# pyannote/pyannote-audio

Measured on NVIDIA H100. Metric: audio-hours/sec (RTF) community-1 diarization, 16kHz mono, 1/2/4/8 H100, higher is better.
Workload: dtype f16 tensor-core trunk (f32 accumulate) + split-f16x3 tensor-core segmentation (f32-level accuracy) + f64 clustering

## Files before the change

pyannote_audio_b200/csrc/emb_conv.cu:

```cuda
#include "common.cuh"
#include "emb.cuh"
#include "tc_common.cuh"

namespace b200 {

constexpr int kWgThreads = 288;
constexpr int kTileM = 128;
constexpr int kRowHalo = 8;
constexpr int kMaxSlots = 16;

template <int N, bool WIDE = false>
__device__ __forceinline__ void conv_epilogue(const float* acc, const ConvParams& p, size_t row, int w0) {
  const int lane = threadIdx.x & 31;
  const int c0 = 2 * (lane & 3) + (WIDE ? (int)blockIdx.y * N : 0);
#pragma unroll
  for (int i = 0; i < 2; ++i) {
    const int w = w0 + ((threadIdx.x >> 5) & 3) * 16 + (lane >> 2) + 8 * i;
    if (w >= p.W_out) continue;
    const size_t pix = (row * p.W_out + w) * (size_t)(WIDE ? p.C_out : N);
    __half2 res[N / 8];
    if (N <= 64 && p.residual) {
#pragma unroll
      for (int j = 0; j < N / 8; ++j) res[j] = *reinterpret_cast<const __half2*>(p.residual + pix + 8 * j + c0);
    }
#pragma unroll
    for (int j = 0; j < N / 8; ++j) {
      const int c = 8 * j + c0;
      const float2 bb = __ldg(reinterpret_cast<const float2*>(p.bias + c));
      float a = acc[4 * j + 2 * i] + bb.x, d = acc[4 * j + 2 * i + 1] + bb.y;
      if (p.residual) {
        const float2 r = __half22float2(N <= 64 ? res[j] : *reinterpret_cast<const __half2*>(p.residual + pix + c));
        a += r.x;
        d += r.y;
      }
      if (p.relu) { a = fmaxf(a, 0.f); d = fmaxf(d, 0.f); }
      *reinterpret_cast<__half2*>(p.out + pix + c) = __floats2half2_rn(a, d);
    }
  }
}

template <int N, int CK, bool WIDE = false>
__global__ void __launch_bounds__(kWgThreads, N == 256 ? 1 : 2)
conv_tc_kernel(const __grid_constant__ CUtensorMap tmA, const __grid_constant__ CUtensorMap tmB, ConvParams p) {
  extern __shared__ uint8_t smem_raw[];
  const uint32_t raw = smem_u32(smem_raw);
  const uint32_t base = (raw + 1023u) & ~1023u;
  const uint32_t bar_full = base, bar_empty = base + 64;
  const uint32_t stage0 = base + 1024;
  const uint32_t stage_bytes = p.a_bytes + p.b_bytes;
  const int warp = threadIdx.x >> 5;
  const int wt = blockIdx.x % p.tiles_w;
  const int bh = blockIdx.x / p.tiles_w;
  const int cchunks = p.C_in / CK;

  if (threadIdx.x == 0) {
    for (uint32_t s = 0; s < p.nstages; ++s) { mbar_init(bar_full + 8 * s, 1); mbar_init(bar_empty + 8 * s, 2); }
    asm volatile("fence.mbarrier_init.release.cluster;" ::: "memory");
  }
  __syncthreads();

  if (warp == 8) {
    if ((threadIdx.x & 31) == 0) {
      prefetch_tensormap(&tmA);
      prefetch_tensormap(&tmB);
      const int h = bh % p.H_out, b = bh / p.H_out;
      const int w_base = wt * kTileM * p.stride - p.pad, h_base = h * p.stride - p.pad;
      uint32_t stage = 0, phase = 0;
      for (int kh = 0; kh < p.taps_h; ++kh)
        for (int kw = 0; kw < p.taps_w; ++kw)
          for (int cc = 0; cc < cchunks; ++cc) {
            mbar_wait(bar_empty + 8 * stage, phase ^ 1);
            mbar_expect_tx(bar_full + 8 * stage, p.a_tx + p.b_bytes);
            const uint32_t sa = stage0 + stage * stage_bytes;
            tma_load_4d(&tmA, bar_full + 8 * stage, sa, cc * CK, w_base + kw, h_base + kh, b);
            tma_load_3d(&tmB, bar_full + 8 * stage, sa + p.a_bytes, cc * CK, WIDE ? (int)blockIdx.y * N : 0,
                        kh * p.taps_w + kw);
            if (++stage == p.nstages) { stage = 0; phase ^= 1; }
          }
    }
    return;
  }

  const int wg = warp >> 2;
  constexpr uint32_t row_bytes = CK * 2;
  float acc[N / 2];
#pragma unroll
  for (int i = 0; i < N / 2; ++i) acc[i] = 0.f;
  const int kblocks = p.taps_h * p.taps_w * cchunks;
  uint32_t stage = 0, phase = 0, prev = 0;
  for (int kb = 0; kb < kblocks; ++kb) {
    mbar_wait(bar_full + 8 * stage, phase);
    const uint32_t st = stage0 + stage * stage_bytes;
    const uint32_t sa = st + (uint32_t)wg * 64u * row_bytes, sb = st + p.a_bytes;
    wg_fence();
    const uint64_t ad = wg_desc(sa, row_bytes), bd = wg_desc(sb, row_bytes);
#pragma unroll
    for (int k = 0; k < CK / 16; ++k) Wgmma<N>::mma(acc, ad + 2 * k, bd + 2 * k);
    wg_commit();
    wg_wait<1>();
    if (kb > 0 && (threadIdx.x & 127) == 0) mbar_arrive(bar_empty + 8 * prev);
    prev = stage;
    if (++stage == p.nstages) { stage = 0; phase ^= 1; }
  }
  wg_wait<0>();
  conv_epilogue<N, WIDE>(acc, p, (size_t)bh, wt * kTileM + wg * 64);
}

template <int N>
__device__ __forceinline__ void row_taps_c32(float (&acc)[2][N / 2], uint32_t sa, uint32_t wts) {
  constexpr uint32_t row_bytes = 64;
  const int warp = threadIdx.x >> 5, lane = threadIdx.x & 31;
#pragma unroll
  for (int kw = 0; kw < 3; ++kw) {
    uint32_t af[2][2][4];
#pragma unroll
    for (int m = 0; m < 2; ++m)
#pragma unroll
      for (int k = 0; k < 2; ++k) {
        const uint32_t row = (uint32_t)(m * 64 + (warp & 3) * 16 + (lane & 15) + kw);
        const uint32_t chunk = (uint32_t)(2 * k + (lane >> 4)) ^ ((row >> 1) & 3u);
        ldsm_x4(af[m][k], sa + row * row_bytes + chunk * 16u);
      }
    wg_fence();
    const uint64_t bd = wg_desc(wts + kw * N * row_bytes, row_bytes);
#pragma unroll
    for (int k = 0; k < 2; ++k)
#pragma unroll
      for (int m = 0; m < 2; ++m) WgmmaRS<N>::mma(acc[m], af[m][k], bd + 2 * k);
    wg_commit();
    wg_wait<0>();
  }
}

template <int N, int CK>
__global__ void __launch_bounds__(kWgThreads, N == 32 ? 2 : 1)
conv_row_kernel(const __grid_constant__ CUtensorMap tmA, const __grid_constant__ CUtensorMap tmB, ConvParams p) {
  constexpr uint32_t row_bytes = CK * 2;
  constexpr uint32_t b_tap_bytes = N * row_bytes;
  extern __shared__ uint8_t smem_raw[];
  const uint32_t base = (smem_u32(smem_raw) + 1023u) & ~1023u;
  const uint32_t bar_w = base, bar_full = base + 8, bar_empty = base + 8 + 8 * kMaxSlots;
  const uint32_t wts = base + 1024;
  const uint32_t slot0 = wts + 9 * b_tap_bytes;
  const uint32_t nslots = p.nstages;
  const int warp = threadIdx.x >> 5;

  if (threadIdx.x == 0) {
    mbar_init(bar_w, 1);
    for (uint32_t s = 0; s < nslots; ++s) { mbar_init(bar_full + 8 * s, 1); mbar_init(bar_empty + 8 * s, 3); }
    asm volatile("fence.mbarrier_init.release.cluster;" ::: "memory");
  }
  __syncthreads();

  if (warp == 8) {
    if ((threadIdx.x & 31) == 0) {
      prefetch_tensormap(&tmA);
      prefetch_tensormap(&tmB);
      mbar_expect_tx(bar_w, 9 * b_tap_bytes);
      for (int kh = 0; kh < 3; ++kh) tma_load_3d(&tmB, bar_w, wts + 3 * kh * b_tap_bytes, 0, 0, 3 * kh);
      uint32_t s = 0;
      for (int u = blockIdx.x; u < p.num_tiles; u += gridDim.x) {
        const int wt = u % p.tiles_w, t = u / p.tiles_w;
        const int h0 = (t % p.bands) * p.band, b = t / p.bands;
        const int n = min(p.band, p.H_out - h0);
        for (int r = 0; r < n + 2; ++r, ++s) {
          const uint32_t slot = s % nslots;
          mbar_wait(bar_empty + 8 * slot, ((s / nslots) & 1) ^ 1);
          mbar_expect_tx(bar_full + 8 * slot, p.a_tx);
          tma_load_4d(&tmA, bar_full + 8 * slot, slot0 + slot * p.a_bytes, 0, wt * kTileM - 1, h0 - 1 + r, b);
        }
      }
    }
    return;
  }

  const int wg = __shfl_sync(0xffffffffu, warp >> 2, 0);
  mbar_wait(bar_w, 0);
  uint32_t s = 0;
  int item = 0;
  for (int u = blockIdx.x; u < p.num_tiles; u += gridDim.x) {
    const int wt = u % p.tiles_w, t = u / p.tiles_w;
    const int h0 = (t % p.bands) * p.band, b = t / p.bands;
    const int n = min(p.band, p.H_out - h0);
    for (int j = 0; j < n; ++j, ++item) {
      if ((item & 1) != wg) continue;
      float acc[2][N / 2];
#pragma unroll
      for (int m = 0; m < 2; ++m)
#pragma unroll
        for (int i = 0; i < N / 2; ++i) {
          acc[m][i] = 0.f;
          asm volatile("" : "+f"(acc[m][i]));
        }
#pragma unroll
      for (int kh = 0; kh < 3; ++kh) {
        const uint32_t q = s + j + kh, slot = q % nslots;
        mbar_wait(bar_full + 8 * slot, (q / nslots) & 1);
        const uint32_t sa = slot0 + slot * p.a_bytes;
        if constexpr (CK == 32) {
          row_taps_c32<N>(acc, sa, wts + 3 * kh * b_tap_bytes);
        } else {
          wg_fence();
#pragma unroll
          for (int kw = 0; kw < 3; ++kw) {
            const uint64_t bd = wg_desc(wts + (3 * kh + kw) * b_tap_bytes, row_bytes);
#pragma unroll
            for (int m = 0; m < 2; ++m) {
              const uint64_t ad = wg_desc(sa + (uint32_t)(m * 64 + kw) * row_bytes, row_bytes);
#pragma unroll
              for (int k = 0; k < CK / 16; ++k) Wgmma<N>::mma(acc[m], ad + 2 * k, bd + 2 * k);
            }
          }
          wg_commit();
        }
      }
      wg_wait<0>();
      if ((threadIdx.x & 127) == 0)
#pragma unroll
        for (int kh = 0; kh < 3; ++kh)
          mbar_arrive_n(bar_empty + 8 * ((s + j + kh) % nslots), 1 + (j == 0 ? 2 - kh : 0) + (j == n - 1 ? kh : 0));
      const size_t row = (size_t)b * p.H_out + h0 + j;
#pragma unroll
      for (int m = 0; m < 2; ++m) conv_epilogue<N>(acc[m], p, row, wt * kTileM + m * 64);
    }
    s += n + 2;
  }
}

struct BlockRowPlan {
  static constexpr uint32_t kTapBytes = 32 * 64;
  static constexpr uint32_t kSlotBytes = 9 * 1024;
  static constexpr uint32_t kInTx = (kTileM + kRowHalo) * 64;
  static constexpr uint32_t kInSlots = 4, kMidSlots = 4;
  static constexpr size_t kSmem = 2048 + 2 * 9 * kTapBytes + (kInSlots + kMidSlots) * kSlotBytes;
  static_assert(kInTx <= kSlotBytes && kSmem <= 113 * 1024, "block row plan");
};
constexpr int kStripW = kTileM - 2;

struct BlockParams {
  int H, W, tiles_w, band, bands, num_tiles;
  const float* bias1;
  const float* bias2;
  __half* out;
};

__device__ __forceinline__ void st_shared_u32(uint32_t a, uint32_t v) {
  asm volatile("st.shared.b32 [%0], %1;" ::"r"(a), "r"(v) : "memory");
}
__device__ __forceinline__ uint32_t ld_shared_u32(uint32_t a) {
  uint32_t v;
  asm volatile("ld.shared.b32 %0, [%1];" : "=r"(v) : "r"(a) : "memory");
  return v;
}
__device__ __forceinline__ uint32_t h2_bits(__half2 h) { return *reinterpret_cast<uint32_t*>(&h); }

__global__ void __launch_bounds__(kWgThreads, 2)
block_row_kernel(const __grid_constant__ CUtensorMap tmA, const __grid_constant__ CUtensorMap tmW1,
                 const __grid_constant__ CUtensorMap tmW2, BlockParams p) {
  using P = BlockRowPlan;
  constexpr uint32_t NI = P::kInSlots, NM = P::kMidSlots;
  extern __shared__ uint8_t smem_raw[];
  const uint32_t base = (smem_u32(smem_raw) + 1023u) & ~1023u;
  const uint32_t bar_w = base, in_full = base + 8, in_empty = in_full + 8 * NI;
  const uint32_t mid_full = in_empty + 8 * NI, mid_empty = mid_full + 8 * NM;
  const uint32_t w1 = base + 1024, w2 = w1 + 9 * P::kTapBytes;
  const uint32_t in0 = w2 + 9 * P::kTapBytes, mid0 = in0 + NI * P::kSlotBytes;
  const int warp = threadIdx.x >> 5, lane = threadIdx.x & 31;

  if (threadIdx.x == 0) {
    mbar_init(bar_w, 1);
    for (uint32_t s = 0; s < NI; ++s) { mbar_init(in_full + 8 * s, 1); mbar_init(in_empty + 8 * s, 4); }
    for (uint32_t s = 0; s < NM; ++s) { mbar_init(mid_full + 8 * s, 128); mbar_init(mid_empty + 8 * s, 3); }
    asm volatile("fence.mbarrier_init.release.cluster;" ::: "memory");
  }
  __syncthreads();

  if (warp == 8) {
    if (lane == 0) {
      prefetch_tensormap(&tmA);
      prefetch_tensormap(&tmW1);
      prefetch_tensormap(&tmW2);
      mbar_expect_tx(bar_w, 18 * P::kTapBytes);
      for (int kh = 0; kh < 3; ++kh) {
        tma_load_3d(&tmW1, bar_w, w1 + 3 * kh * P::kTapBytes, 0, 0, 3 * kh);
        tma_load_3d(&tmW2, bar_w, w2 + 3 * kh * P::kTapBytes, 0, 0, 3 * kh);
      }
      uint32_t s = 0;
      for (int u = blockIdx.x; u < p.num_tiles; u += gridDim.x) {
        const int wt = u % p.tiles_w, t = u / p.tiles_w;
        const int h0 = (t % p.bands) * p.band, b = t / p.bands;
        const int n = min(p.band, p.H - h0);
        for (int r = 0; r < n + 4; ++r, ++s) {
          const uint32_t slot = s % NI;
          mbar_wait(in_empty + 8 * slot, ((s / NI) & 1) ^ 1);
          mbar_expect_tx(in_full + 8 * slot, P::kInTx);
          tma_load_4d(&tmA, in_full + 8 * slot, in0 + slot * P::kSlotBytes, 0, wt * kStripW - 2, h0 - 2 + r, b);
        }
      }
    }
    return;
  }

  const int wg = __shfl_sync(0xffffffffu, warp >> 2, 0);
  const bool leader = (threadIdx.x & 127) == 0;
  const int c0 = 2 * (lane & 3);
  float2 bias[4];
#pragma unroll
  for (int j = 0; j < 4; ++j) bias[j] = __ldg(reinterpret_cast<const float2*>((wg ? p.bias2 : p.bias1) + 8 * j + c0));
  mbar_wait(bar_w, 0);
  uint32_t s = 0, mq = 0;
  for (int u = blockIdx.x; u < p.num_tiles; u += gridDim.x) {
    const int wt = u % p.tiles_w, t = u / p.tiles_w;
    const int h0 = (t % p.bands) * p.band, b = t / p.bands;
    const int n = min(p.band, p.H - h0);
    const int w0 = wt * kStripW;
    const int rows = wg == 0 ? n + 2 : n;
    for (int j = 0; j < rows; ++j) {
      float acc[2][16];
#pragma unroll
      for (int m = 0; m < 2; ++m)
#pragma unroll
        for (int i = 0; i < 16; ++i) {
          acc[m][i] = 0.f;
          asm volatile("" : "+f"(acc[m][i]));
        }
      if (wg == 0) {
#pragma unroll
        for (int kh = 0; kh < 3; ++kh) {
          const uint32_t q = s + j + kh, slot = q % NI;
          mbar_wait(in_full + 8 * slot, (q / NI) & 1);
          row_taps_c32<32>(acc, in0 + slot * P::kSlotBytes, w1 + 3 * kh * P::kTapBytes);
        }
        if (leader)
#pragma unroll
          for (int kh = 0; kh < 3; ++kh) {
            const int k = j + kh;
            const bool no_res = (k < 2 || k >= n + 2) && j == min(k, n + 1);
            mbar_arrive_n(in_empty + 8 * ((s + k) % NI),
                          1 + (j == 0 ? 2 - kh : 0) + (j == n + 1 ? kh : 0) + (no_res ? 1 : 0));
          }
        const uint32_t q = mq + j, slot = q % NM, sm = mid0 + slot * P::kSlotBytes;
        mbar_wait(mid_empty + 8 * slot, ((q / NM) & 1) ^ 1);
        const int r = h0 - 1 + j;
        const bool live = r >= 0 && r < p.H;
#pragma unroll
        for (int m = 0; m < 2; ++m)
#pragma unroll
          for (int i = 0; i < 2; ++i) {
            const int px = m * 64 + (warp & 3) * 16 + (lane >> 2) + 8 * i, w = w0 - 1 + px;
            const bool in = live && w >= 0 && w < p.W;
#pragma unroll
            for (int jj = 0; jj < 4; ++jj) {
              const float a = fmaxf(acc[m][4 * jj + 2 * i] + bias[jj].x, 0.f);
              const float d = fmaxf(acc[m][4 * jj + 2 * i + 1] + bias[jj].y, 0.f);
              const uint32_t v = in ? h2_bits(__floats2half2_rn(a, d)) : 0u;
              st_shared_u32(sm + px * 64u + ((jj ^ ((px >> 1) & 3)) << 4) + 2 * c0, v);
            }
          }
        mbar_arrive(mid_full + 8 * slot);
      } else {
#pragma unroll
        for (int kh = 0; kh < 3; ++kh) {
          const uint32_t q = mq + j + kh, slot = q % NM;
          mbar_wait(mid_full + 8 * slot, (q / NM) & 1);
          row_taps_c32<32>(acc, mid0 + slot * P::kSlotBytes, w2 + 3 * kh * P::kTapBytes);
        }
        if (leader)
#pragma unroll
          for (int kh = 0; kh < 3; ++kh)
            mbar_arrive_n(mid_empty + 8 * ((mq + j + kh) % NM), 1 + (j == 0 ? 2 - kh : 0) + (j == n - 1 ? kh : 0));
        const uint32_t q = s + j + 2, slot = q % NI, sr = in0 + slot * P::kSlotBytes;
        mbar_wait(in_full + 8 * slot, (q / NI) & 1);
        const size_t row = (size_t)b * p.H + h0 + j;
#pragma unroll
        for (int m = 0; m < 2; ++m)
#pragma unroll
          for (int i = 0; i < 2; ++i) {
            const int px = m * 64 + (warp & 3) * 16 + (lane >> 2) + 8 * i, w = w0 + px;
            if (px >= kStripW || w >= p.W) continue;
            const int rp = px + 2;
            __half2* o = reinterpret_cast<__half2*>(p.out + (row * p.W + w) * 32 + c0);
#pragma unroll
            for (int jj = 0; jj < 4; ++jj) {
              const uint32_t rb = ld_shared_u32(sr + rp * 64u + ((jj ^ ((rp >> 1) & 3)) << 4) + 2 * c0);
              const float2 rv = __half22float2(*reinterpret_cast<const __half2*>(&rb));
              float a = acc[m][4 * jj + 2 * i] + bias[jj].x, d = acc[m][4 * jj + 2 * i + 1] + bias[jj].y;
              a += rv.x;
              d += rv.y;
              o[4 * jj] = __floats2half2_rn(fmaxf(a, 0.f), fmaxf(d, 0.f));
            }
          }
        asm volatile("bar.sync 1, 128;" ::: "memory");
        if (leader) mbar_arrive(in_empty + 8 * slot);
      }
    }
    s += n + 4;
    mq += n + 2;
  }
}

template <int N>
struct ChunkRowPlan {
  static constexpr int kChunks = N / 64;
  static constexpr int kCtasPerSm = N == 256 ? 1 : 2;
  static constexpr uint32_t kABytes = (kTileM + kRowHalo) * 128;
  static constexpr uint32_t kBBytes = N * 128;
  static constexpr uint32_t kASlots = N == 256 ? 5 : 3;
  static constexpr uint32_t kBSlots = N == 256 ? 4 : 3;
  static constexpr size_t kSmem = 2048 + kASlots * kABytes + kBSlots * kBBytes;
  static_assert(kASlots > kChunks && kASlots <= 8 && kBSlots <= 8, "chunk row ring plan");
};

template <int N>
__global__ void __launch_bounds__(kWgThreads, ChunkRowPlan<N>::kCtasPerSm)
conv_chunk_row_kernel(const __grid_constant__ CUtensorMap tmA, const __grid_constant__ CUtensorMap tmB, ConvParams p) {
  using P = ChunkRowPlan<N>;
  constexpr int CH = P::kChunks, KSTEPS = 9 * CH;
  extern __shared__ uint8_t smem_raw[];
  const uint32_t base = (smem_u32(smem_raw) + 1023u) & ~1023u;
  const uint32_t full_a = base, empty_a = base + 64, full_b = base + 128, empty_b = base + 192;
  const uint32_t ring_a = base + 1024, ring_b = ring_a + P::kASlots * P::kABytes;
  const int warp = threadIdx.x >> 5;

  if (threadIdx.x == 0) {
    for (uint32_t s = 0; s < P::kASlots; ++s) { mbar_init(full_a + 8 * s, 1); mbar_init(empty_a + 8 * s, 2); }
    for (uint32_t s = 0; s < P::kBSlots; ++s) { mbar_init(full_b + 8 * s, 1); mbar_init(empty_b + 8 * s, 2); }
    asm volatile("fence.mbarrier_init.release.cluster;" ::: "memory");
  }
  __syncthreads();

  if (warp == 8) {
    if ((threadIdx.x & 31) == 0) {
      prefetch_tensormap(&tmA);
      prefetch_tensormap(&tmB);
      uint32_t qa = 0, qb = 0;
      for (int u = blockIdx.x; u < p.num_tiles; u += gridDim.x) {
        const int wt = u % p.tiles_w, t = u / p.tiles_w;
        const int h = t % p.H_out, b = t / p.H_out;
        for (int s = 0; s < KSTEPS; ++s) {
          const int cc = s % CH, kw = (s / CH) % 3, kh = s / (3 * CH);
          if (kw == 0) {
            const uint32_t q = qa + kh * CH + cc, slot = q % P::kASlots;
            mbar_wait(empty_a + 8 * slot, ((q / P::kASlots) & 1) ^ 1);
            mbar_expect_tx(full_a + 8 * slot, P::kABytes);
            tma_load_4d(&tmA, full_a + 8 * slot, ring_a + slot * P::kABytes, cc * 64, wt * kTileM - 1, h - 1 + kh, b);
          }
          const uint32_t q = qb + s, slot = q % P::kBSlots;
          mbar_wait(empty_b + 8 * slot, ((q / P::kBSlots) & 1) ^ 1);
          mbar_expect_tx(full_b + 8 * slot, P::kBBytes);
          tma_load_3d(&tmB, full_b + 8 * slot, ring_b + slot * P::kBBytes, cc * 64, 0, 3 * kh + kw);
        }
        qa += 3 * CH;
        qb += KSTEPS;
      }
    }
    return;
  }

  const int wg = __shfl_sync(0xffffffffu, warp >> 2, 0);
  const bool leader = (threadIdx.x & 127) == 0;
  uint32_t qa = 0, qb = 0;
  for (int u = blockIdx.x; u < p.num_tiles; u += gridDim.x) {
    const int wt = u % p.tiles_w, t = u / p.tiles_w;
    const int h = t % p.H_out, b = t / p.H_out;
    float acc[N / 2];
#pragma unroll
    for (int i = 0; i < N / 2; ++i) {
      acc[i] = 0.f;
      asm volatile("" : "+f"(acc[i]));
    }
    uint32_t prev_b = 0, prev_a = 0;
    bool prev_frees_a = false;
    auto release = [&]() {
      if (leader) {
        mbar_arrive(empty_b + 8 * prev_b);
        if (prev_frees_a) mbar_arrive(empty_a + 8 * prev_a);
      }
    };
    for (int s = 0; s < KSTEPS; ++s) {
      const int cc = s % CH, kw = (s / CH) % 3, kh = s / (3 * CH);
      const uint32_t qA = qa + kh * CH + cc, sa = qA % P::kASlots;
      const uint32_t qB = qb + s, sb = qB % P::kBSlots;
      mbar_wait(full_a + 8 * sa, (qA / P::kASlots) & 1);
      mbar_wait(full_b + 8 * sb, (qB / P::kBSlots) & 1);
      wg_fence();
      const uint64_t ad = wg_desc(ring_a + sa * P::kABytes + (uint32_t)(wg * 64 + kw) * 128u, 128);
      const uint64_t bd = wg_desc(ring_b + sb * P::kBBytes, 128);
#pragma unroll
      for (int k = 0; k < 4; ++k) Wgmma<N>::mma(acc, ad + 2 * k, bd + 2 * k);
      wg_commit();
      wg_wait<1>();
      if (s > 0) release();
      prev_b = sb;
      prev_a = sa;
      prev_frees_a = kw == 2;
    }
    wg_wait<0>();
    release();
    qa += 3 * CH;
    qb += KSTEPS;
    conv_epilogue<N>(acc, p, (size_t)b * p.H_out + h, wt * kTileM + wg * 64);
  }
}

__global__ void conv_simt_kernel(const __half* __restrict__ in, const __half* __restrict__ wt, ConvParams p) {
  const int groups = p.C_out / 8;
  const size_t idx = (size_t)blockIdx.x * blockDim.x + threadIdx.x;
  const size_t total = (size_t)p.B * p.H_out * p.W_out * groups;
  if (idx >= total) return;
  const int g = idx % groups;
  size_t pixel = idx / groups;
  const int w = pixel % p.W_out;
  const int h = (pixel / p.W_out) % p.H_out;
  const int b = pixel / ((size_t)p.W_out * p.H_out);
  float acc[8];
#pragma unroll
  for (int j = 0; j < 8; ++j) acc[j] = p.bias[g * 8 + j];
  for (int kh = 0; kh < p.taps_h; ++kh) {
    const int hi = h * p.stride + kh - p.pad;
    if (hi < 0 || hi >= p.H_in) continue;
    for (int kw = 0; kw < p.taps_w; ++kw) {
      const int wi = w * p.stride + kw - p.pad;
      if (wi < 0 || wi >= p.W_in) continue;
      const __half* ip = in + (((size_t)b * p.H_in + hi) * p.W_in + wi) * p.C_in;
      const int tap = kh * p.taps_w + kw;
      for (int ci = 0; ci < p.C_in; ci += 8) {
        uint4 xu = *reinterpret_cast<const uint4*>(ip + ci);
        const __half2* xh = reinterpret_cast<const __half2*>(&xu);
        float x[8];
#pragma unroll
        for (int e = 0; e < 4; ++e) {
          float2 f = __half22float2(xh[e]);
          x[2 * e] = f.x;
          x[2 * e + 1] = f.y;
        }
#pragma unroll
        for (int j = 0; j < 8; ++j) {
          uint4 wu = *reinterpret_cast<const uint4*>(wt + ((size_t)tap * p.C_out + g * 8 + j) * p.C_in + ci);
          const __half2* wh = reinterpret_cast<const __half2*>(&wu);
#pragma unroll
          for (int e = 0; e < 4; ++e) {
            float2 f = __half22float2(wh[e]);
            acc[j] = fmaf(x[2 * e], f.x, acc[j]);
            acc[j] = fmaf(x[2 * e + 1], f.y, acc[j]);
          }
        }
      }
    }
  }
  const size_t o = (((size_t)b * p.H_out + h) * p.W_out + w) * p.C_out + g * 8;
  if (p.residual) {
    uint4 ru = *reinterpret_cast<const uint4*>(p.residual + o);
    const __half2* rh = reinterpret_cast<const __half2*>(&ru);
#pragma unroll
    for (int e = 0; e < 4; ++e) {
      float2 f = __half22float2(rh[e]);
      acc[2 * e] += f.x;
      acc[2 * e + 1] += f.y;
    }
  }
  uint4 ou;
  __half2* oh = reinterpret_cast<__half2*>(&ou);
#pragma unroll
  for (int e = 0; e < 4; ++e) {
    float a = acc[2 * e], c = acc[2 * e + 1];
    if (p.relu) { a = fmaxf(a, 0.f); c = fmaxf(c, 0.f); }
    oh[e] = __floats2half2_rn(a, c);
  }
  *reinterpret_cast<uint4*>(p.out + o) = ou;
}

constexpr int kC1Tile = 128;
__global__ void __launch_bounds__(kC1Tile) conv1_kernel(const float* __restrict__ fbank, const float* __restrict__ fmean,
                             const int* __restrict__ frame0, const float* __restrict__ w , const float* __restrict__ bias ,
                             __half* __restrict__ out, int T0) {
  __shared__ __align__(16) float sw[9 * 32];
  __shared__ __align__(16) float sb[32];
  __shared__ float sx[(kC1Tile + 2) * (kMel + 1)];
  const int b = blockIdx.x, t0 = blockIdx.y * kC1Tile;
  const size_t r0 = frame0 ? (size_t)frame0[b] : (size_t)b * T0;
  for (int i = threadIdx.x; i < 288; i += blockDim.x) sw[(i % 9) * 32 + i / 9] = w[i];
  if (threadIdx.x < 32) sb[threadIdx.x] = bias[threadIdx.x];
  for (int i = threadIdx.x; i < (kC1Tile + 2) * kMel; i += blockDim.x) {
    const int tt = i / kMel, f = i - tt * kMel;
    const int t = t0 - 1 + tt;
    float v = 0.f;
    if (t >= 0 && t < T0) v = fbank[(r0 + t) * kMel + f] - fmean[(size_t)b * kMel + f];
    sx[tt * (kMel + 1) + f] = v;
  }
  __syncthreads();
  const int t = t0 + threadIdx.x;
  if (t >= T0) return;
  const float* col = sx + threadIdx.x * (kMel + 1);
  for (int h = 0; h < kMel; ++h) {
    asm volatile("" ::: "memory");
    float x[9];
#pragma unroll
    for (int kh = 0; kh < 3; ++kh) {
      const int hh = h + kh - 1;
      const bool ok = hh >= 0 && hh < kMel;
#pragma unroll
      for (int kw = 0; kw < 3; ++kw) x[kh * 3 + kw] = ok ? col[kw * (kMel + 1) + hh] : 0.f;
    }
    f32x2_t acc2[16];
    const ulonglong2* sb2 = reinterpret_cast<const ulonglong2*>(sb);
#pragma unroll
    for (int q = 0; q < 8; ++q) { const ulonglong2 bb = sb2[q]; acc2[2 * q] = bb.x; acc2[2 * q + 1] = bb.y; }
#pragma unroll
    for (int k = 0; k < 9; ++k) {
      const f32x2_t xk = pack2(x[k], x[k]);
      const ulonglong2* wk = reinterpret_cast<const ulonglong2*>(sw + k * 32);
#pragma unroll
      for (int q = 0; q < 8; ++q) {
        const ulonglong2 w4 = wk[q];
        ffma2(acc2[2 * q], xk, w4.x);
        ffma2(acc2[2 * q + 1], xk, w4.y);
      }
    }
    __half2 o[16];
#pragma unroll
    for (int c = 0; c < 16; ++c) {
      float a0, a1;
      unpack2(acc2[c], a0, a1);
      o[c] = __floats2half2_rn(fmaxf(a0, 0.f), fmaxf(a1, 0.f));
    }
    uint4* op = reinterpret_cast<uint4*>(out + (((size_t)b * kMel + h) * T0 + t) * 32);
    const uint4* src = reinterpret_cast<const uint4*>(o);
#pragma unroll
    for (int i = 0; i < 4; ++i) op[i] = src[i];
  }
}

typedef CUresult (*PFN_encodeTiled)(CUtensorMap*, CUtensorMapDataType, cuuint32_t, void*, const cuuint64_t*,
                                    const cuuint64_t*, const cuuint32_t*, const cuuint32_t*, CUtensorMapInterleave,
                                    CUtensorMapSwizzle, CUtensorMapL2promotion, CUtensorMapFloatOOBfill);

static PFN_encodeTiled get_encode() {
  static PFN_encodeTiled fn = nullptr;
  if (!fn) {
    void* ptr = nullptr;
    cudaDriverEntryPointQueryResult qres;
    if (cudaGetDriverEntryPoint("cuTensorMapEncodeTiled", &ptr, cudaEnableDefault, &qres) == cudaSuccess &&
        qres == cudaDriverEntryPointSuccess)
      fn = reinterpret_cast<PFN_encodeTiled>(ptr);
  }
  return fn;
}

int encode_f16_map(CUtensorMap* tm, int rank, const void* ptr, const cuuint64_t* dims, const cuuint64_t* strides,
                   const cuuint32_t* box, const cuuint32_t* estr, CUtensorMapSwizzle swizzle, const char* what) {
  PFN_encodeTiled enc = get_encode();
  B200_CHECK(enc != nullptr, B200_ERR_CUDA, "cuTensorMapEncodeTiled not available from the driver");
  const cuuint32_t ones[5] = {1, 1, 1, 1, 1};
  CUresult r = enc(tm, CU_TENSOR_MAP_DATA_TYPE_FLOAT16, (cuuint32_t)rank, const_cast<void*>(ptr), dims, strides, box,
                   estr ? estr : ones, CU_TENSOR_MAP_INTERLEAVE_NONE, swizzle, CU_TENSOR_MAP_L2_PROMOTION_L2_256B,
                   CU_TENSOR_MAP_FLOAT_OOB_FILL_NONE);
  B200_CHECK(r == CUDA_SUCCESS, B200_ERR_CUDA, "cuTensorMapEncodeTiled(%s) failed: %d", what, (int)r);
  return B200_OK;
}

int conv_forward(const ConvLayer& L, const __half* in, const __half* residual, __half* out, int B, int H_in, int W_in,
                 int relu, int impl, int num_sms, cudaStream_t stream) {
  ConvParams p{};
  p.B = B; p.H_in = H_in; p.W_in = W_in; p.C_in = L.C_in; p.C_out = L.C_out;
  p.taps_h = L.ksize; p.taps_w = L.ksize; p.stride = L.stride; p.pad = L.ksize / 2;
  p.H_out = (H_in + 2 * p.pad - L.ksize) / L.stride + 1;
  p.W_out = (W_in + 2 * p.pad - L.ksize) / L.stride + 1;
  p.relu = relu; p.bias = L.bias; p.residual = residual; p.out = out;
  p.Ck = (L.C_in >= 64) ? 64 : 32;
  p.swizzle = (p.Ck == 64) ? 128 : 64;
  p.tiles_w = ceil_div(p.W_out, kTileM);
  p.num_tiles = B * p.H_out * p.tiles_w;
  B200_CHECK(L.C_in % p.Ck == 0 && (L.C_out == 32 || L.C_out == 64 || L.C_out == 128 ||
                                    (L.C_out % 256 == 0 && L.C_out <= 1024 && p.Ck == 64)),
             B200_ERR_STATE, "conv %d -> %d channels unsupported", L.C_in, L.C_out);
  const int n_tile = std::min(L.C_out, 256);
  B200_CHECK(impl >= 0 && impl <= 2, B200_ERR_INVALID,
             "conv_impl %d unknown (0 = CUDA cores, 1 = tensor cores, 2 = tensor cores, one weight tap per stage)", impl);

  if (impl == 0) {
    const size_t total = (size_t)B * p.H_out * p.W_out * (L.C_out / 8);
    conv_simt_kernel<<<(unsigned)((total + 255) / 256), 256, 0, stream>>>(in, L.w, p);
    B200_CUDA_OK(cudaGetLastError());
    return B200_OK;
  }

  const bool rows = impl == 1 && L.ksize == 3 && L.stride == 1 && L.C_in == p.Ck && L.C_out == L.C_in;
  const bool chunk_rows =
      impl == 1 && L.ksize == 3 && L.stride == 1 && L.C_out == L.C_in && (L.C_out == 128 || L.C_out == 256);
  p.a_rows = rows || chunk_rows ? kTileM + kRowHalo : kTileM;
  p.a_tx = p.a_rows * p.Ck * 2;
  p.a_bytes = (p.a_tx + 1023u) & ~1023u;
  size_t smem;
  int ctas = 0;
  if (rows) {
    const int per_sm = L.C_out == 32 ? 2 : 1;
    const size_t budget = per_sm == 2 ? 113u * 1024 : 227u * 1024;
    const size_t fixed = 2048 + (size_t)9 * L.C_out * p.Ck * 2;
    p.nstages = (uint32_t)std::min<size_t>(kMaxSlots, (budget - fixed) / p.a_bytes);
    B200_CHECK(p.nstages >= 6, B200_ERR_STATE, "conv %d -> %d: row ring too shallow", L.C_in, L.C_out);
    smem = fixed + (size_t)p.nstages * p.a_bytes;
    ctas = per_sm * num_sms;
    const int strips = B * p.tiles_w;
    const int nbands = std::min(p.H_out, ceil_div(ctas, strips));
    p.band = ceil_div(p.H_out, nbands);
    p.bands = ceil_div(p.H_out, p.band);
    p.num_tiles = strips * p.bands;
  } else if (chunk_rows) {
    smem = L.C_out == 256 ? ChunkRowPlan<256>::kSmem : ChunkRowPlan<128>::kSmem;
    ctas = (L.C_out == 256 ? ChunkRowPlan<256>::kCtasPerSm : ChunkRowPlan<128>::kCtasPerSm) * num_sms;
  } else {
    p.b_bytes = (uint32_t)(n_tile * p.Ck * 2);
    const uint32_t budget = n_tile == 256 ? 200u * 1024 : 100u * 1024;
    p.nstages = std::min(budget / (p.a_bytes + p.b_bytes), 8u);
    B200_CHECK(p.nstages >= 2, B200_ERR_STATE, "conv %d -> %d: shared memory plan too shallow", L.C_in, L.C_out);
    smem = 1024 + 1024 + (size_t)p.nstages * (p.a_bytes + p.b_bytes);
  }
  const CUtensorMapSwizzle swz = p.swizzle == 128 ? CU_TENSOR_MAP_SWIZZLE_128B : CU_TENSOR_MAP_SWIZZLE_64B;
  CUtensorMap tmA, tmB;
  int rc;
  {
    const cuuint64_t dims[4] = {(cuuint64_t)L.C_in, (cuuint64_t)W_in, (cuuint64_t)H_in, (cuuint64_t)B};
    const cuuint64_t strides[3] = {(cuuint64_t)L.C_in * 2, (cuuint64_t)W_in * L.C_in * 2,
                                   (cuuint64_t)H_in * W_in * L.C_in * 2};
    const cuuint32_t box[4] = {(cuuint32_t)p.Ck, (cuuint32_t)(p.a_rows * L.stride), 1, 1};
    const cuuint32_t estr[4] = {1, (cuuint32_t)L.stride, 1, 1};
    if ((rc = encode_f16_map(&tmA, 4, in, dims, strides, box, estr, swz, "A"))) return rc;
  }
  {
    const cuuint64_t dims[3] = {(cuuint64_t)L.C_in, (cuuint64_t)L.C_out, (cuuint64_t)(L.ksize * L.ksize)};
    const cuuint64_t strides[2] = {(cuuint64_t)L.C_in * 2, (cuuint64_t)L.C_out * L.C_in * 2};
    const cuuint32_t box[3] = {(cuuint32_t)p.Ck, (cuuint32_t)n_tile, rows ? 3u : 1u};
    if ((rc = encode_f16_map(&tmB, 3, L.w, dims, strides, box, nullptr, swz, "B"))) return rc;
  }
  auto launch = [&](auto kernel) -> int {
    B200_CUDA_OK(cudaFuncSetAttribute(kernel, cudaFuncAttributeMaxDynamicSharedMemorySize, (int)smem));
    const dim3 grid((unsigned)(ctas ? std::min(p.num_tiles, ctas) : p.num_tiles), (unsigned)(L.C_out / n_tile));
    kernel<<<grid, kWgThreads, smem, stream>>>(tmA, tmB, p);
    B200_CUDA_OK(cudaGetLastError());
    return B200_OK;
  };
  if (rows) return p.Ck == 32 ? launch(conv_row_kernel<32, 32>) : launch(conv_row_kernel<64, 64>);
  if (chunk_rows) return L.C_out == 256 ? launch(conv_chunk_row_kernel<256>) : launch(conv_chunk_row_kernel<128>);
  if (p.Ck == 32) {
    switch (L.C_out) {
      case 32: return launch(conv_tc_kernel<32, 32>);
      case 64: return launch(conv_tc_kernel<64, 32>);
      default: return launch(conv_tc_kernel<128, 32>);
    }
  }
  switch (L.C_out) {
    case 32: return launch(conv_tc_kernel<32, 64>);
    case 64: return launch(conv_tc_kernel<64, 64>);
    case 128: return launch(conv_tc_kernel<128, 64>);
    case 256: return launch(conv_tc_kernel<256, 64>);
    default: return launch(conv_tc_kernel<256, 64, true>);
  }
}

bool block_fused(const BlockWeights& Bw, int impl) {
  return impl == 1 && !Bw.has_shortcut && Bw.conv1.stride == 1 && Bw.conv1.ksize == 3 && Bw.conv2.ksize == 3 &&
         Bw.conv1.C_in == 32 && Bw.conv1.C_out == 32 && Bw.conv2.C_in == 32 && Bw.conv2.C_out == 32;
}

int block_forward(const BlockWeights& Bw, const __half* in, __half* out, int B, int H, int W, int num_sms,
                  cudaStream_t stream) {
  B200_CHECK(block_fused(Bw, 1), B200_ERR_STATE, "block %d -> %d (stride %d) has no fused kernel", Bw.conv1.C_in,
             Bw.conv1.C_out, Bw.conv1.stride);
  B200_CHECK(in != out, B200_ERR_INVALID, "fused block: output must not alias the input");
  BlockParams p{};
  p.H = H; p.W = W; p.bias1 = Bw.conv1.bias; p.bias2 = Bw.conv2.bias; p.out = out;
  p.tiles_w = ceil_div(W, kStripW);
  const int ctas = 2 * num_sms;
  const int strips = B * p.tiles_w;
  const int nbands = std::min(H, ceil_div(ctas, strips));
  p.band = ceil_div(H, nbands);
  p.bands = ceil_div(H, p.band);
  p.num_tiles = strips * p.bands;
  CUtensorMap tmA, tmW1, tmW2;
  int rc;
  {
    const cuuint64_t dims[4] = {32, (cuuint64_t)W, (cuuint64_t)H, (cuuint64_t)B};
    const cuuint64_t strides[3] = {64, (cuuint64_t)W * 64, (cuuint64_t)H * W * 64};
    const cuuint32_t box[4] = {32, kTileM + kRowHalo, 1, 1};
    if ((rc = encode_f16_map(&tmA, 4, in, dims, strides, box, nullptr, CU_TENSOR_MAP_SWIZZLE_64B, "block A"))) return rc;
  }
  {
    const cuuint64_t dims[3] = {32, 32, 9};
    const cuuint64_t strides[2] = {64, 32 * 64};
    const cuuint32_t box[3] = {32, 32, 3};
    if ((rc = encode_f16_map(&tmW1, 3, Bw.conv1.w, dims, strides, box, nullptr, CU_TENSOR_MAP_SWIZZLE_64B, "block W1")))
      return rc;
    if ((rc = encode_f16_map(&tmW2, 3, Bw.conv2.w, dims, strides, box, nullptr, CU_TENSOR_MAP_SWIZZLE_64B, "block W2")))
      return rc;
  }
  const size_t smem = BlockRowPlan::kSmem;
  B200_CUDA_OK(cudaFuncSetAttribute(block_row_kernel, cudaFuncAttributeMaxDynamicSharedMemorySize, (int)smem));
  block_row_kernel<<<(unsigned)std::min(p.num_tiles, ctas), kWgThreads, smem, stream>>>(tmA, tmW1, tmW2, p);
  B200_CUDA_OK(cudaGetLastError());
  return B200_OK;
}

int conv1_forward(const float* fbank, const float* fmean, const int* frame0, const float* w, const float* bias,
                  __half* out, int B, int T0, cudaStream_t stream) {
  dim3 grid(B, ceil_div(T0, kC1Tile));
  conv1_kernel<<<grid, kC1Tile, 0, stream>>>(fbank, fmean, frame0, w, bias, out, T0);
  B200_CUDA_OK(cudaGetLastError());
  return B200_OK;
}

}
```

Before: 1.592.

## Process two output rows per CTA in chunk-row conv to share halo and weight tiles

For the 128-channel chunk-row conv, each CTA now computes two adjacent output rows, one per warpgroup. Each warpgroup covers the full 128-wide tile with two M-halves, so weight tiles and the overlapping input rows are loaded once and used by both rows. To fit the larger rings the kernel drops to one CTA per SM. It also prefetches residual rows into L2 before the epilogue and loads the residual into registers for N up to 128. The risk is lower occupancy, twice the accumulator registers per thread, and more complex ring slot accounting.

```diff
diff --git a/pyannote_audio_b200/csrc/emb_conv.cu b/pyannote_audio_b200/csrc/emb_conv.cu
--- a/pyannote_audio_b200/csrc/emb_conv.cu
+++ b/pyannote_audio_b200/csrc/emb_conv.cu
@@ -9,17 +9,19 @@
 constexpr int kRowHalo = 8;
 constexpr int kMaxSlots = 16;
 
-template <int N, bool WIDE = false>
+template <int N, bool WIDE = false, int MH = 1>
 __device__ __forceinline__ void conv_epilogue(const float* acc, const ConvParams& p, size_t row, int w0) {
   const int lane = threadIdx.x & 31;
   const int c0 = 2 * (lane & 3) + (WIDE ? (int)blockIdx.y * N : 0);
 #pragma unroll
+  for (int m = 0; m < MH; ++m)
+#pragma unroll
   for (int i = 0; i < 2; ++i) {
-    const int w = w0 + ((threadIdx.x >> 5) & 3) * 16 + (lane >> 2) + 8 * i;
+    const int w = w0 + 64 * m + ((threadIdx.x >> 5) & 3) * 16 + (lane >> 2) + 8 * i;
     if (w >= p.W_out) continue;
     const size_t pix = (row * p.W_out + w) * (size_t)(WIDE ? p.C_out : N);
     __half2 res[N / 8];
-    if (N <= 64 && p.residual) {
+    if (N <= 128 && p.residual) {
 #pragma unroll
       for (int j = 0; j < N / 8; ++j) res[j] = *reinterpret_cast<const __half2*>(p.residual + pix + 8 * j + c0);
     }
@@ -27,9 +29,9 @@
     for (int j = 0; j < N / 8; ++j) {
       const int c = 8 * j + c0;
       const float2 bb = __ldg(reinterpret_cast<const float2*>(p.bias + c));
-      float a = acc[4 * j + 2 * i] + bb.x, d = acc[4 * j + 2 * i + 1] + bb.y;
+      float a = acc[m * (N / 2) + 4 * j + 2 * i] + bb.x, d = acc[m * (N / 2) + 4 * j + 2 * i + 1] + bb.y;
       if (p.residual) {
-        const float2 r = __half22float2(N <= 64 ? res[j] : *reinterpret_cast<const __half2*>(p.residual + pix + c));
+        const float2 r = __half22float2(N <= 128 ? res[j] : *reinterpret_cast<const __half2*>(p.residual + pix + c));
         a += r.x;
         d += r.y;
       }
@@ -402,20 +404,26 @@
 template <int N>
 struct ChunkRowPlan {
   static constexpr int kChunks = N / 64;
-  static constexpr int kCtasPerSm = N == 256 ? 1 : 2;
+  static constexpr int kRows = N == 128 ? 2 : 1;
+  static constexpr int kHalves = N == 128 ? 2 : 1;
   static constexpr uint32_t kABytes = (kTileM + kRowHalo) * 128;
   static constexpr uint32_t kBBytes = N * 128;
-  static constexpr uint32_t kASlots = N == 256 ? 5 : 3;
-  static constexpr uint32_t kBSlots = N == 256 ? 4 : 3;
+  static constexpr uint32_t kASlots = N == 256 ? 5 : 8;
+  static constexpr uint32_t kBSlots = N == 256 ? 4 : 5;
   static constexpr size_t kSmem = 2048 + kASlots * kABytes + kBSlots * kBBytes;
-  static_assert(kASlots > kChunks && kASlots <= 8 && kBSlots <= 8, "chunk row ring plan");
+  static_assert(kASlots >= kRows * kChunks + 1 && kASlots <= 8 && kBSlots <= 8, "chunk row ring plan");
+  static_assert(kSmem <= 227 * 1024, "chunk row shared memory");
+  __device__ __forceinline__ static uint32_t box(int r, int cc) {
+    return r < kRows ? cc * kRows + r : kRows * kChunks + (r - kRows) * kChunks + cc;
+  }
 };
 
 template <int N>
-__global__ void __launch_bounds__(kWgThreads, ChunkRowPlan<N>::kCtasPerSm)
+__global__ void __launch_bounds__(kWgThreads, 1)
 conv_chunk_row_kernel(const __grid_constant__ CUtensorMap tmA, const __grid_constant__ CUtensorMap tmB, ConvParams p) {
   using P = ChunkRowPlan<N>;
-  constexpr int CH = P::kChunks, KSTEPS = 9 * CH;
+  constexpr int CH = P::kChunks, R = P::kRows, KSTEPS = 9 * CH;
+  constexpr uint32_t BOXES = (R + 2) * CH;
   extern __shared__ uint8_t smem_raw[];
   const uint32_t base = (smem_u32(smem_raw) + 1023u) & ~1023u;
   const uint32_t full_a = base, empty_a = base + 64, full_b = base + 128, empty_b = base + 192;
@@ -436,21 +444,22 @@
       uint32_t qa = 0, qb = 0;
       for (int u = blockIdx.x; u < p.num_tiles; u += gridDim.x) {
         const int wt = u % p.tiles_w, t = u / p.tiles_w;
-        const int h = t % p.H_out, b = t / p.H_out;
+        const int h = (t % p.bands) * R, b = t / p.bands;
         for (int s = 0; s < KSTEPS; ++s) {
           const int cc = s % CH, kw = (s / CH) % 3, kh = s / (3 * CH);
-          if (kw == 0) {
-            const uint32_t q = qa + kh * CH + cc, slot = q % P::kASlots;
-            mbar_wait(empty_a + 8 * slot, ((q / P::kASlots) & 1) ^ 1);
-            mbar_expect_tx(full_a + 8 * slot, P::kABytes);
-            tma_load_4d(&tmA, full_a + 8 * slot, ring_a + slot * P::kABytes, cc * 64, wt * kTileM - 1, h - 1 + kh, b);
-          }
+          if (kw == 0)
+            for (int r = kh == 0 ? 0 : kh + R - 1; r < kh + R; ++r) {
+              const uint32_t q = qa + P::box(r, cc), slot = q % P::kASlots;
+              mbar_wait(empty_a + 8 * slot, ((q / P::kASlots) & 1) ^ 1);
+              mbar_expect_tx(full_a + 8 * slot, P::kABytes);
+              tma_load_4d(&tmA, full_a + 8 * slot, ring_a + slot * P::kABytes, cc * 64, wt * kTileM - 1, h - 1 + r, b);
+            }
           const uint32_t q = qb + s, slot = q % P::kBSlots;
           mbar_wait(empty_b + 8 * slot, ((q / P::kBSlots) & 1) ^ 1);
           mbar_expect_tx(full_b + 8 * slot, P::kBBytes);
           tma_load_3d(&tmB, full_b + 8 * slot, ring_b + slot * P::kBBytes, cc * 64, 0, 3 * kh + kw);
         }
-        qa += 3 * CH;
+        qa += BOXES;
         qb += KSTEPS;
       }
     }
@@ -459,47 +468,62 @@
 
   const int wg = __shfl_sync(0xffffffffu, warp >> 2, 0);
   const bool leader = (threadIdx.x & 127) == 0;
+  const int ro = R == 2 ? wg : 0;
   uint32_t qa = 0, qb = 0;
   for (int u = blockIdx.x; u < p.num_tiles; u += gridDim.x) {
     const int wt = u % p.tiles_w, t = u / p.tiles_w;
-    const int h = t % p.H_out, b = t / p.H_out;
-    float acc[N / 2];
-#pragma unroll
-    for (int i = 0; i < N / 2; ++i) {
-      acc[i] = 0.f;
-      asm volatile("" : "+f"(acc[i]));
-    }
-    uint32_t prev_b = 0, prev_a = 0;
-    bool prev_frees_a = false;
+    const int h = (t % p.bands) * R + ro, b = t / p.bands;
+    const int w0 = wt * kTileM + (R == 2 ? 0 : wg * 64);
+    if (p.residual && h < p.H_out)
+#pragma unroll
+      for (int l = (threadIdx.x & 127); l < 256; l += 128) {
+        const int w = w0 + l / (N / 64);
+        if (w < p.W_out)
+          asm volatile("prefetch.global.L2 [%0];" ::"l"(p.residual + ((size_t)(b * p.H_out + h) * p.W_out + w) * N +
+                                                         (l % (N / 64)) * 64));
+      }
+    float acc[P::kHalves][N / 2];
+#pragma unroll
+    for (int m = 0; m < P::kHalves; ++m)
+#pragma unroll
+      for (int i = 0; i < N / 2; ++i) {
+        acc[m][i] = 0.f;
+        asm volatile("" : "+f"(acc[m][i]));
+      }
+    uint32_t prev_b = 0, prev_a = 0, prev_frees_a = 0;
     auto release = [&]() {
       if (leader) {
         mbar_arrive(empty_b + 8 * prev_b);
-        if (prev_frees_a) mbar_arrive(empty_a + 8 * prev_a);
+        if (prev_frees_a) mbar_arrive_n(empty_a + 8 * prev_a, prev_frees_a);
       }
     };
     for (int s = 0; s < KSTEPS; ++s) {
       const int cc = s % CH, kw = (s / CH) % 3, kh = s / (3 * CH);
-      const uint32_t qA = qa + kh * CH + cc, sa = qA % P::kASlots;
+      const uint32_t qA = qa + P::box(kh + ro, cc), sa = qA % P::kASlots;
       const uint32_t qB = qb + s, sb = qB % P::kBSlots;
       mbar_wait(full_a + 8 * sa, (qA / P::kASlots) & 1);
       mbar_wait(full_b + 8 * sb, (qB / P::kBSlots) & 1);
       wg_fence();
-      const uint64_t ad = wg_desc(ring_a + sa * P::kABytes + (uint32_t)(wg * 64 + kw) * 128u, 128);
       const uint64_t bd = wg_desc(ring_b + sb * P::kBBytes, 128);
 #pragma unroll
-      for (int k = 0; k < 4; ++k) Wgmma<N>::mma(acc, ad + 2 * k, bd + 2 * k);
+      for (int m = 0; m < P::kHalves; ++m) {
+        const uint32_t half = R == 2 ? m : wg;
+        const uint64_t ad = wg_desc(ring_a + sa * P::kABytes + (half * 64 + kw) * 128u, 128);
+#pragma unroll
+        for (int k = 0; k < 4; ++k) Wgmma<N>::mma(acc[m], ad + 2 * k, bd + 2 * k);
+      }
       wg_commit();
       wg_wait<1>();
       if (s > 0) release();
       prev_b = sb;
       prev_a = sa;
-      prev_frees_a = kw == 2;
+      prev_frees_a = kw == 2 ? (R == 2 && kh == 2 * ro ? 2 : 1) : 0;
     }
     wg_wait<0>();
     release();
-    qa += 3 * CH;
+    qa += BOXES;
     qb += KSTEPS;
-    conv_epilogue<N>(acc, p, (size_t)b * p.H_out + h, wt * kTileM + wg * 64);
+    if (h < p.H_out) conv_epilogue<N, false, P::kHalves>(acc[0], p, (size_t)b * p.H_out + h, w0);
   }
 }
 
@@ -707,8 +731,11 @@
     p.bands = ceil_div(p.H_out, p.band);
     p.num_tiles = strips * p.bands;
   } else if (chunk_rows) {
+    p.band = L.C_out == 256 ? ChunkRowPlan<256>::kRows : ChunkRowPlan<128>::kRows;
+    p.bands = ceil_div(p.H_out, p.band);
+    p.num_tiles = B * p.bands * p.tiles_w;
     smem = L.C_out == 256 ? ChunkRowPlan<256>::kSmem : ChunkRowPlan<128>::kSmem;
-    ctas = (L.C_out == 256 ? ChunkRowPlan<256>::kCtasPerSm : ChunkRowPlan<128>::kCtasPerSm) * num_sms;
+    ctas = num_sms;
   } else {
     p.b_bytes = (uint32_t)(n_tile * p.Ck * 2);
     const uint32_t budget = n_tile == 256 ? 200u * 1024 : 100u * 1024;
```

After: 1.668 (median of 6 runs). +4.8%, better.
